# UBC-AWP/vision-sam3-yolo-lameless

Hardware: AMD Instinct MI355X
Metric: frames/sec (whole node) for YOLO+SAM3+DINOv3 feature extraction, 1080p clips (higher is better)
Workload: dtype f16; 1 GPU; BASELINE cfg#5, dense schedule: fused per-frame path on a synthetic 5 s @ 30 fps 1080p clip (150 unique BGR frames resident in HBM): YOLOv8-l detect (letterbox 384x640, NMS, scale_boxes; f16 plan) -> SAM (Hiera-B+ image encoder + FPN at 1024x1024, box-prompted mask decoder, 1080p mask + statistics + contour features) + DINOv3 ViT-L/16 embed (224x224) on EVERY frame; per-frame records packed, gathe; parallelism=one clip per GPU, 1 GPU(s), one gather per step, streams=7

## Files before the change

### vision-sam3-yolo-lameless_amd/csrc/attn.hip

```cpp
#include "common.h"
#include <type_traits>
#include <stdlib.h>

#ifdef LMX_DBG_TIMELINE
__device__ unsigned long long lmx_attn_tl[64 * 8 * 8];
extern "C" int lmx_dbg_get_attn_timeline(void* host, int64_t bytes) { return (int)hipMemcpyFromSymbol(host, HIP_SYMBOL(lmx_attn_tl), bytes); }
#define ATL(i) if (blockIdx.x == 0 && lane == 0 && tl_it < 64) lmx_attn_tl[(tl_it * 8 + wave) * 8 + (i)] = __builtin_readcyclecounter()
#else
#define ATL(i)
#endif
namespace {

struct Geo {
  int mode, Tq, Tk, Gh, Gw, ws, nWy, nWx, Gqh, Gqw, wsq;
};

__device__ __forceinline__ int64_t key_row(const Geo& g, int b, int t) {
  if (g.mode == 0) return (int64_t)b * g.Tk + t;
  const int nW = g.nWy * g.nWx;
  const int img = b / nW;
  const int w = b - img * nW;
  const int wy = w / g.nWx, wx = w - wy * g.nWx;
  const int ty = t / g.ws, tx = t - ty * g.ws;
  const int y = wy * g.ws + ty, x = wx * g.ws + tx;
// ... 691 lines not shown
  const int hd = p.hd;
  const half8_t zero8 = {0, 0, 0, 0, 0, 0, 0, 0};

  {
    const int r = lane >> 2, c0 = (lane & 3) * 2;
    const bool in = r < p.Tk;
    const int64_t row = key_row(geo, b, in ? r : 0);
    const bool pad = row < 0;
    half_t* dst = &Vs[wave][r * 64];
#pragma unroll
    for (int e = 0; e < 2; ++e) {
      const int c = c0 + e, d = c * 8;
      const bool ok = in && d < hd && (!pad || padv);
      const half_t* vp = (in && d < hd) ? (pad ? (padv ? padv + (int64_t)h * hd + d : V) : V + row * p.ldv + (int64_t)h * hd + d) : V;
      const half8_t vv = *reinterpret_cast<const half8_t*>(vp);
      *reinterpret_cast<half8_t*>(dst + ((c ^ (r & 7)) << 3)) = ok ? vv : zero8;
    }
  }
  const int64_t qrow = fr < p.Tq ? query_row(geo, b, fr) : -1;
  const bool kin = fr < p.Tk;
  const int64_t krow = key_row(geo, b, kin ? fr : 0);
  const bool kpad = krow < 0;
  half8_t qf[2], kf[2];
#pragma unroll
  for (int ks = 0; ks < 2; ++ks) {
    const int d = ks * 32 + fg * 8;
    const bool dq = qrow >= 0 && d < hd;
    const half8_t qv = *reinterpret_cast<const half8_t*>(Q + (dq ? qrow * p.ldq + (int64_t)h * hd + d : 0));
    qf[ks] = dq ? qv : zero8;
    const bool dk = kin && d < hd;
    const half_t* kp = dk ? (kpad ? (padk ? padk + (int64_t)h * hd + d : K) : K + krow * p.ldk + (int64_t)h * hd + d) : K;
    const half8_t kv = *reinterpret_cast<const half8_t*>(kp);
    kf[ks] = (dk && (!kpad || padk)) ? kv : zero8;
  }
  f32x4 sacc = {0.f, 0.f, 0.f, 0.f};
  sacc = __builtin_amdgcn_mfma_f32_16x16x32_f16(kf[0], qf[0], sacc, 0, 0, 0);
  sacc = __builtin_amdgcn_mfma_f32_16x16x32_f16(kf[1], qf[1], sacc, 0, 0, 0);
  const float sl2 = p.scale * 1.44269504088896340736f;
#pragma unroll
  for (int i = 0; i < 4; ++i)
    if (fg * 4 + i >= p.Tk) sacc[i] = -INFINITY;
  float mx = fmaxf(fmaxf(sacc[0], sacc[1]), fmaxf(sacc[2], sacc[3]));
  mx = fmaxf(mx, __shfl_xor(mx, 16, 64));
  mx = fmaxf(mx, __shfl_xor(mx, 32, 64));
  const float mb = mx * sl2;
  half8_t pf = zero8;
  float l = 0.f;
#pragma unroll
  for (int i = 0; i < 4; ++i) {
    const half_t e = (half_t)__builtin_amdgcn_exp2f(fmaf(sacc[i], sl2, -mb));
    pf[i] = e;
    l += (float)e;
  }
  l += __shfl_xor(l, 16, 64);
  l += __shfl_xor(l, 32, 64);
  const float inv = 1.0f / l;
  const int q4 = fr >> 2, p4 = fr & 3;
  const int r0 = fg * 4 + q4;
  half_t* O = reinterpret_cast<half_t*>(p.O);
#pragma unroll
  for (int db = 0; db < 4; ++db) {
    const int chunk = db * 2 + (p4 >> 1);
    const half4_t lo = lds_tr_read(&Vs[wave][r0 * 64 + ((chunk ^ (r0 & 7)) << 3) + (p4 & 1) * 4]);
    const half8_t vf = {lo[0], lo[1], lo[2], lo[3], 0, 0, 0, 0};
    f32x4 oacc = {0.f, 0.f, 0.f, 0.f};
    oacc = __builtin_amdgcn_mfma_f32_16x16x32_f16(vf, pf, oacc, 0, 0, 0);
    const int d = db * 16 + fg * 4;
    if (qrow >= 0 && d < hd) {
      const half4_t o = {(half_t)(oacc[0] * inv), (half_t)(oacc[1] * inv), (half_t)(oacc[2] * inv), (half_t)(oacc[3] * inv)};
      *reinterpret_cast<half4_t*>(O + qrow * p.ldo + (int64_t)h * hd + d) = o;
    }
  }
}

template <int KS>
__global__ __launch_bounds__(256) void relpos_tables_kernel(const lmx_attn_desc p, const Geo geo, const float* __restrict__ rh,
                                                            const float* __restrict__ rw, int S, half_t* __restrict__ out,
                                                            const int64_t items) {
  const int lane = threadIdx.x & 63, wave = threadIdx.x >> 6;
  const int fr = lane & 15, fg = lane >> 4;
  const int64_t item = (int64_t)blockIdx.x * 4 + wave;
  if (item >= items) return;
  const int line = (int)(item % S);
  const int axis = (int)((item / S) & 1);
  const int64_t bh = item / (2 * S);
  const int h = (int)(bh % p.H), b = (int)(bh / p.H);
  const int hd = p.hd;
  const float* R = axis ? rw : rh;
  const half_t* Q = reinterpret_cast<const half_t*>(p.Q);
  const half8_t zero8 = {0, 0, 0, 0, 0, 0, 0, 0};
  const int nblk = (S + 15) / 16;
  for (int mb = 0; mb < nblk; ++mb) {
    const int pos = mb * 16 + fr;
    const int t = axis ? pos * S + line : line * S + pos;
    const int64_t qrow = pos < S ? query_row(geo, b, t) : -1;
    half8_t qf[KS];
#pragma unroll
    for (int ks = 0; ks < KS; ++ks) {
      const int d = ks * 32 + fg * 8;
      const bool ok = qrow >= 0 && d < hd;
      const half8_t qv = *reinterpret_cast<const half8_t*>(Q + (ok ? qrow * p.ldq + (int64_t)h * hd + d : 0));
      qf[ks] = ok ? qv : zero8;
    }
    half_t* orow = out + ((bh * p.Tq) + (pos < S ? t : 0)) * (2 * S) + axis * S;
    for (int jb = 0; jb < nblk; ++jb) {
      const int j = jb * 16 + fr;
      f32x4 acc = {0.f, 0.f, 0.f, 0.f};
#pragma unroll
      for (int ks = 0; ks < KS; ++ks) {
        const int d = ks * 32 + fg * 8;
        const bool ok = j < S && d < hd;
        const float* rp = R + (ok ? (int64_t)(line - j + S - 1) * hd + d : 0);
        const f32x4 r0 = *reinterpret_cast<const f32x4*>(rp), r1 = *reinterpret_cast<const f32x4*>(rp + (ok ? 4 : 0));
        const half8_t rf = {(half_t)r0[0], (half_t)r0[1], (half_t)r0[2], (half_t)r0[3],
                            (half_t)r1[0], (half_t)r1[1], (half_t)r1[2], (half_t)r1[3]};
        acc = __builtin_amdgcn_mfma_f32_16x16x32_f16(ok ? rf : zero8, qf[ks], acc, 0, 0, 0);
      }
      const int j0 = jb * 16 + fg * 4;
      if (pos < S && j0 < S) {
        if (j0 + 3 < S && (S & 3) == 0) {
          const half4_t o = {(half_t)acc[0], (half_t)acc[1], (half_t)acc[2], (half_t)acc[3]};
          *reinterpret_cast<half4_t*>(orow + j0) = o;
        } else {
          for (int i = 0; i < 4 && j0 + i < S; ++i) orow[j0 + i] = (half_t)acc[i];
        }
      }
    }
  }
}


template <int QB, bool ONES>
__global__ __launch_bounds__(256, QB == 2 ? 2 : 3) void attn_sp_kernel(const lmx_attn_desc p, const Geo geo) {
  constexpr int RW = 64, CPR = 8, KB = 13, KROWS = KB * 16, VROWS = KROWS, NPASS = (KROWS + 31) / 32;
  __shared__ __attribute__((aligned(16))) half_t Ks[KROWS * RW];
  __shared__ __attribute__((aligned(16))) half_t Vs[VROWS * RW];
  const int tid = threadIdx.x, lane = tid & 63, wave = tid >> 6;
  const int fr = lane & 15, fg = lane >> 4;
  int bid;
  {
    const int n = gridDim.x, xcd = blockIdx.x & 7, idx = blockIdx.x >> 3, q = n >> 3, r = n & 7;
    bid = (xcd < r ? xcd * (q + 1) : r * (q + 1) + (xcd - r) * q) + idx;
  }
  const int h = bid % p.H, b = bid / p.H;
  const half_t* Q = reinterpret_cast<const half_t*>(p.Q);
  const half_t* K = reinterpret_cast<const half_t*>(p.K);
  const half_t* V = reinterpret_cast<const half_t*>(p.V);
  const half_t* padk = reinterpret_cast<const half_t*>(p.pad_k);
  const half_t* padv = reinterpret_cast<const half_t*>(p.pad_v);
  half_t* O = reinterpret_cast<half_t*>(p.O);
  const int hd = p.hd;
  const half8_t zero8 = {0, 0, 0, 0, 0, 0, 0, 0};

  {
    const int sc = tid & (CPR - 1), sk = tid / CPR;
    const int d = sc * 8;
    const int64_t hoff = (int64_t)h * hd + d;
#pragma unroll
    for (int half = 0; half < 2; ++half) {
      constexpr int H0 = 4;
      half8_t kst[H0], vst[H0];
#pragma unroll
      for (int j = 0; j < H0; ++j) {
        const int i = half * H0 + j;
        if (i >= NPASS) continue;
        const int t = sk + 32 * i;
        const bool in = (t < p.Tk) && (d < hd);
        const int64_t row = geo.mode == 0 ? (int64_t)b * p.Tk + (in ? t : 0) : key_row(geo, b, in ? t : 0);
        const bool pad = row < 0;
        const half_t* kp = pad ? (padk ? padk + hoff : K) : K + (in ? row * p.ldk + hoff : 0);
        const half_t* vp = pad ? (padv ? padv + hoff : V) : V + (in ? row * p.ldv + hoff : 0);
        const half8_t kv = *reinterpret_cast<const half8_t*>(kp);
        const half8_t vv = *reinterpret_cast<const half8_t*>(vp);
        kst[j] = (in && (!pad || padk)) ? kv : zero8;
        vst[j] = (in && (!pad || padv)) ? vv : zero8;
        if (ONES && sc == 7 && t < p.Tk) vst[j][7] = (half_t)1.0f;
      }
#pragma unroll
      for (int j = 0; j < H0; ++j) {
        const int i = half * H0 + j;
        if (i >= NPASS) continue;
        const int kk = sk + 32 * i;
        const int off = kk * RW + ((sc ^ (kk & (CPR - 1))) << 3);
        if (kk < KROWS) {
          *reinterpret_cast<half8_t*>(&Ks[off]) = kst[j];
          *reinterpret_cast<half8_t*>(&Vs[off]) = vst[j];
        }
      }
    }
  }
  __syncthreads();

  const float sl2 = p.scale * 1.44269504088896340736f;
  const int q4 = fr >> 2, p4 = fr & 3;
  const int nqb = (p.Tq + 15) / 16, npair = (nqb + QB - 1) / QB;
  for (int pr = wave; pr < npair; pr += 4) {
    half8_t qf[QB][2];
    int64_t qrow[QB];
#pragma unroll
    for (int qb = 0; qb < QB; ++qb) {
      const int tq = (pr * QB + qb) * 16 + fr;
      qrow[qb] = (tq < p.Tq) ? query_row(geo, b, tq) : -1;
#pragma unroll
      for (int ks = 0; ks < 2; ++ks) {
        const int d = ks * 32 + fg * 8;
        const bool ok = qrow[qb] >= 0 && d < hd;
        const half8_t qv = *reinterpret_cast<const half8_t*>(Q + (ok ? qrow[qb] * p.ldq + (int64_t)h * hd + d : 0));
        qf[qb][ks] = ok ? qv : zero8;
      }
    }
    f32x4 sacc[QB][KB];
#pragma unroll
    for (int qb = 0; qb < QB; ++qb)
#pragma unroll
      for (int kb = 0; kb < KB; ++kb) sacc[qb][kb] = f32x4{0.f, 0.f, 0.f, 0.f};
#pragma unroll
    for (int ks = 0; ks < 2; ++ks) {
      const int coff = (((ks << 2) + fg) ^ (fr & (CPR - 1))) << 3;
#pragma unroll
      for (int kb = 0; kb < KB; ++kb) {
        const half8_t kf = *reinterpret_cast<const half8_t*>(&Ks[(kb * 16 + fr) * RW + coff]);
#pragma unroll
        for (int qb = 0; qb < QB; ++qb) sacc[qb][kb] = __builtin_amdgcn_mfma_f32_16x16x32_f16(kf, qf[qb][ks], sacc[qb][kb], 0, 0, 0);
      }
    }
    half8_t pf[QB][7];
    float l_sum[QB];
#pragma unroll
    for (int qb = 0; qb < QB; ++qb) {
#pragma unroll
      for (int kb = 8; kb < KB; ++kb)
#pragma unroll
        for (int r = 0; r < 4; ++r)
          if (kb * 16 + fg * 4 + r >= p.Tk) sacc[qb][kb][r] = -INFINITY;
      float mx = fmaxf(fmaxf(sacc[qb][0][0], sacc[qb][0][1]), fmaxf(sacc[qb][0][2], sacc[qb][0][3]));
#pragma unroll
      for (int kb = 1; kb < KB; ++kb)
        mx = fmaxf(mx, fmaxf(fmaxf(sacc[qb][kb][0], sacc[qb][kb][1]), fmaxf(sacc[qb][kb][2], sacc[qb][kb][3])));
      mx = fmaxf(mx, __shfl_xor(mx, 16, 64));
      mx = fmaxf(mx, __shfl_xor(mx, 32, 64));
      const float mb = mx * sl2;
      float rs = 0.f;
      const half2_t ones2 = {(half_t)1.0f, (half_t)1.0f};
#pragma unroll
      for (int kb = 0; kb < KB + 1; ++kb)
#pragma unroll
        for (int r = 0; r < 4; r += 2) {
          half2_t e = {(half_t)0.0f, (half_t)0.0f};
          if (kb < KB) {
            const float e0 = __builtin_amdgcn_exp2f(fmaf(sacc[qb][kb][r], sl2, -mb));
            const float e1 = __builtin_amdgcn_exp2f(fmaf(sacc[qb][kb][r + 1], sl2, -mb));
            e = half2_t{(half_t)e0, (half_t)e1};
            if (!ONES) rs = __builtin_amdgcn_fdot2(e, ones2, rs, false);
          }
          pf[qb][kb >> 1][(kb & 1) * 4 + r] = e[0];
          pf[qb][kb >> 1][(kb & 1) * 4 + r + 1] = e[1];
        }
      l_sum[qb] = rs;
    }
    f32x4 oacc[QB][4];
#pragma unroll
    for (int qb = 0; qb < QB; ++qb)
#pragma unroll
      for (int db = 0; db < 4; ++db) oacc[qb][db] = f32x4{0.f, 0.f, 0.f, 0.f};
#pragma unroll
    for (int ks = 0; ks < 7; ++ks) {
#pragma unroll
      for (int db = 0; db < 4; ++db) {
        const int chunk = db * 2 + (p4 >> 1);
        const int r0 = ks * 32 + fg * 4 + q4, r1 = ks == 6 ? r0 : r0 + 16;
        const half4_t lo = lds_tr_read(&Vs[r0 * RW + ((chunk ^ (r0 & (CPR - 1))) << 3) + (p4 & 1) * 4]);
        const half4_t hi = lds_tr_read(&Vs[r1 * RW + ((chunk ^ (r1 & (CPR - 1))) << 3) + (p4 & 1) * 4]);
        const half8_t vf = {lo[0], lo[1], lo[2], lo[3], hi[0], hi[1], hi[2], hi[3]};
#pragma unroll
        for (int qb = 0; qb < QB; ++qb) oacc[qb][db] = __builtin_amdgcn_mfma_f32_16x16x32_f16(vf, pf[qb][ks], oacc[qb][db], 0, 0, 0);
      }
    }
#pragma unroll
    for (int qb = 0; qb < QB; ++qb) {
      float l;
      if (ONES) {
        l = __shfl(oacc[qb][3][3], 48 + fr, 64);
      } else {
        l = l_sum[qb];
        l += __shfl_xor(l, 16, 64);
        l += __shfl_xor(l, 32, 64);
      }
      const float inv = 1.0f / l;
      if (qrow[qb] < 0) continue;
#pragma unroll
      for (int db = 0; db < 4; ++db) {
        const int d = db * 16 + fg * 4;
        if (d >= hd) continue;
        half4_t o;
#pragma unroll
        for (int r = 0; r < 4; ++r) o[r] = (half_t)(oacc[qb][db][r] * inv);
        *reinterpret_cast<half4_t*>(O + qrow[qb] * p.ldo + (int64_t)h * hd + d) = o;
      }
    }
  }
}


template <bool ONES>
__global__ __launch_bounds__(512, 1) void attn_spp_kernel(const lmx_attn_desc p, const Geo geo, const int items) {
  constexpr int RW = 64, CPR = 8, KB = 13, ROWS = KB * 16, QB = 2, NWV = 8;
  constexpr int TEN = ROWS * RW * 2;
  constexpr int BUF = 3 * TEN;
  extern __shared__ __attribute__((aligned(16))) char smem[];
  const int tid = threadIdx.x, lane = tid & 63;
  const int wave = __builtin_amdgcn_readfirstlane(tid >> 6);
  const int fr = lane & 15, fg = lane >> 4;
  const int hd = p.hd, H_ = p.H, Tq_ = p.Tq, Tk_ = p.Tk, mode_ = geo.mode;
  const int64_t ldq_ = p.ldq, ldk_ = p.ldk, ldv_ = p.ldv;
  const int ws_ = geo.ws, wsq_ = geo.wsq, Gh_ = geo.Gh, Gw_ = geo.Gw, Gqh_ = geo.Gqh, Gqw_ = geo.Gqw, nWx_ = geo.nWx, nW_ = geo.nWy * geo.nWx;

  {
    const u32x4 z = {0u, 0u, 0u, 0u};
    for (int i = tid; i < 2 * BUF / 16; i += 512) *reinterpret_cast<u32x4*>(smem + i * 16) = z;
    __syncthreads();
    if (ONES)
      for (int i = tid; i < 2 * ROWS; i += 512) {
        const int bsel = i / ROWS, row = i - bsel * ROWS;
        half_t* v = reinterpret_cast<half_t*>(smem + bsel * BUF + 2 * TEN);
        v[row * RW + ((7 ^ (row & 7)) << 3) + 7] = (half_t)1.0f;
      }
  }

  const int xcd = blockIdx.x & 7, jx = blockIdx.x >> 3;
  const int nwg = ((int)gridDim.x + 7 - xcd) >> 3;
  const int iq = items >> 3, ir = items & 7;
  const int ibase = xcd < ir ? xcd * (iq + 1) : ir * (iq + 1) + (xcd - ir) * iq;
  const int icnt = iq + (xcd < ir ? 1 : 0);

  constexpr int NJ = 4;
  unsigned rel[3][NJ];
  int tyx[3][NJ];
#pragma unroll
  for (int ten = 0; ten < 3; ++ten)
#pragma unroll
    for (int m = 0; m < NJ; ++m) {
      const int j = wave + NWV * m;
      const int row = 8 * j + (lane >> 3);
      const int lc = (lane & 7) ^ (row & 7);
      const int d = lc * 8;
      const int T = ten == 0 ? Tq_ : Tk_;
      const int wsz = ten == 0 ? wsq_ : ws_;
      const int gw = ten == 0 ? Gqw_ : Gw_;
      const int64_t ld = ten == 0 ? ldq_ : (ten == 1 ? ldk_ : ldv_);
      const int ty = mode_ == 0 ? 0 : row / wsz, tx = mode_ == 0 ? row : row - ty * wsz;
      rel[ten][m] = (unsigned)((((int64_t)(mode_ == 0 ? row : ty * gw + tx)) * ld + d) * 2);
      tyx[ten][m] = ((j < 26 && row < T && d < hd) ? (1 << 30) : 0) | (d << 20) | (ty << 10) | tx;
    }
  const char* Qg = reinterpret_cast<const char*>(p.Q);
  const char* Kg = reinterpret_cast<const char*>(p.K);
  const char* Vg = reinterpret_cast<const char*>(p.V);
  const char* padk = reinterpret_cast<const char*>(p.pad_k);
  const char* padv = reinterpret_cast<const char*>(p.pad_v);
  int qty[QB], qtx[QB];
#pragma unroll
  for (int qb = 0; qb < QB; ++qb) {
    const int tq = (wave * QB + qb) * 16 + fr;
    qty[qb] = mode_ == 0 ? 0 : tq / wsq_;
    qtx[qb] = mode_ == 0 ? tq : tq - qty[qb] * wsq_;
  }

  auto issue = [&](int item, int bsel) {
    const int h = item % H_, b = item / H_;
    int img = b, wy = 0, wx = 0;
    if (mode_ != 0) {
      img = b / nW_;
      const int w = b - img * nW_;
      wy = w / nWx_;
      wx = w - wy * nWx_;
    }
    const int64_t hcol = (int64_t)h * hd * 2;
    const char *oq, *ok, *ov;
    int qy = 1 << 20, qx = 1 << 20, ky = 1 << 20, kx = 1 << 20;
    if (mode_ == 0) {
      oq = Qg + (int64_t)b * Tq_ * ldq_ * 2 + hcol;
      ok = Kg + (int64_t)b * Tk_ * ldk_ * 2 + hcol;
      ov = Vg + (int64_t)b * Tk_ * ldv_ * 2 + hcol;
    } else {
      const int64_t q0 = ((int64_t)img * Gqh_ + wy * wsq_) * Gqw_ + wx * wsq_;
      const int64_t k0 = ((int64_t)img * Gh_ + wy * ws_) * Gw_ + wx * ws_;
      oq = Qg + q0 * ldq_ * 2 + hcol;
      ok = Kg + k0 * ldk_ * 2 + hcol;
      ov = Vg + k0 * ldv_ * 2 + hcol;
      qy = Gqh_ - wy * wsq_, qx = Gqw_ - wx * wsq_, ky = Gh_ - wy * ws_, kx = Gw_ - wx * ws_;
    }
    const bool edge = qy < wsq_ || qx < wsq_ || ky < ws_ || kx < ws_;
    char* base = smem + bsel * BUF + wave * 1024;
#pragma unroll
    for (int ten = 0; ten < 3; ++ten) {
      const char* org = ten == 0 ? oq : (ten == 1 ? ok : ov);
      const char* pv = (ten == 1 ? padk : padv) + hcol;
#pragma unroll
      for (int m = 0; m < NJ; ++m) {
        if (wave + NWV * m >= 26) break;
        const int pl = tyx[ten][m];
        bool act = (pl >> 30) & 1;
        const char* src = org + rel[ten][m];
        if (edge) {
          const int ty = (pl >> 10) & 1023, tx = pl & 1023;
          if (ten == 0) {
            act = act && ty < qy && tx < qx;
          } else if (ty >= ky || tx >= kx) {
            src = pv + ((pl >> 20) & 1023) * 2;
          }
        }
        char* dst = base + ten * TEN + m * (NWV * 1024);
        if (act) __builtin_amdgcn_global_load_lds(reinterpret_cast<const void*>(src), (lds_ptr_t)dst, 16, 0, 0);
      }
    }
  };

  const float sl2 = p.scale * 1.44269504088896340736f;
  const int q4 = fr >> 2, p4 = fr & 3;
  const int nqb = (Tq_ + 15) / 16, npair = (nqb + QB - 1) / QB;
  __syncthreads();
  const bool early = wave < NWV / 2;
  if (jx < icnt) issue(ibase + jx, 0);
  asm volatile("s_waitcnt vmcnt(0)" ::: "memory");
  int bsel = 0;
#ifdef LMX_DBG_TIMELINE
  int tl_it = -1;
#endif
  for (int li = jx; li < icnt; li += nwg, bsel ^= 1) {
    const int item = ibase + li;
    const int h = item % p.H, b = item / p.H;
#ifdef LMX_DBG_TIMELINE
    ++tl_it;
#endif
    ATL(0);
    __syncthreads();
    ATL(1);
    const bool more = li + nwg < icnt;
    if (more && (early || wave >= npair)) issue(item + nwg, bsel ^ 1);
    ATL(2);
    const half_t* Qs = reinterpret_cast<const half_t*>(smem + bsel * BUF);
    const half_t* Ks = Qs + ROWS * RW;
    const half_t* Vs = Ks + ROWS * RW;
    const int pr = wave;
    if (pr < npair) {
      half8_t qf[QB][2];
      int64_t qrow[QB];
#pragma unroll
      for (int qb = 0; qb < QB; ++qb) {
        const int tq = (pr * QB + qb) * 16 + fr;
        if (mode_ == 0) {
          qrow[qb] = tq < Tq_ ? (int64_t)b * Tq_ + tq : -1;
        } else {
          const int img = b / nW_, w = b - img * nW_;
          const int wy = w / nWx_, wx = w - wy * nWx_;
          const int y = wy * wsq_ + qty[qb], x = wx * wsq_ + qtx[qb];
          qrow[qb] = (tq < Tq_ && y < Gqh_ && x < Gqw_) ? ((int64_t)img * Gqh_ + y) * Gqw_ + x : -1;
        }
        const int lr = tq < ROWS ? tq : ROWS - 1;
#pragma unroll
        for (int ks = 0; ks < 2; ++ks) qf[qb][ks] = *reinterpret_cast<const half8_t*>(&Qs[lr * RW + ((((ks << 2) + fg) ^ (lr & 7)) << 3)]);
      }
      f32x4 sacc[QB][KB];
#pragma unroll
      for (int qb = 0; qb < QB; ++qb)
#pragma unroll
        for (int kb = 0; kb < KB; ++kb) sacc[qb][kb] = f32x4{0.f, 0.f, 0.f, 0.f};
      {
        auto kread = [&](int i) {
          const int ks = i / KB, kb = i - ks * KB;
          return *reinterpret_cast<const half8_t*>(&Ks[(kb * 16 + fr) * RW + ((((ks << 2) + fg) ^ (fr & (CPR - 1))) << 3)]);
        };
        half8_t kring[3];
        kring[0] = kread(0);
        kring[1] = kread(1);
#pragma unroll
        for (int i = 0; i < 2 * KB; ++i) {
          if (i + 2 < 2 * KB) kring[(i + 2) % 3] = kread(i + 2);
          __builtin_amdgcn_sched_barrier(0);
          const int ks = i / KB, kb = i - ks * KB;
#pragma unroll
          for (int qb = 0; qb < QB; ++qb) sacc[qb][kb] = __builtin_amdgcn_mfma_f32_16x16x32_f16(kring[i % 3], qf[qb][ks], sacc[qb][kb], 0, 0, 0);
          __builtin_amdgcn_sched_barrier(0);
        }
      }
      if (more && !early) issue(item + nwg, bsel ^ 1);
      ATL(3);
      half8_t pf[QB][7];
      float l_sum[QB];
#pragma unroll
      for (int qb = 0; qb < QB; ++qb) {
#pragma unroll
        for (int kb = 8; kb < KB; ++kb)
          if (kb * 16 + 16 > Tk_) {
#pragma unroll
            for (int r = 0; r < 4; ++r)
              if (kb * 16 + fg * 4 + r >= Tk_) sacc[qb][kb][r] = -INFINITY;
          }
        float ma = vmax3(sacc[qb][0][0], sacc[qb][0][1], sacc[qb][0][2]);
        float mc = vmax3(sacc[qb][0][3], sacc[qb][1][0], sacc[qb][1][1]);
        ma = vmax3(ma, sacc[qb][1][2], sacc[qb][1][3]);
#pragma unroll
        for (int kb = 2; kb < KB; ++kb) {
          if (kb & 1)
            ma = vmax3(ma, sacc[qb][kb][0], sacc[qb][kb][1]), ma = vmax3(ma, sacc[qb][kb][2], sacc[qb][kb][3]);
          else
            mc = vmax3(mc, sacc[qb][kb][0], sacc[qb][kb][1]), mc = vmax3(mc, sacc[qb][kb][2], sacc[qb][kb][3]);
        }
        const float mx = row_max4(ma, mc);
        const float mb = mx * sl2;
        float rs = 0.f;
        const half2_t ones2 = {(half_t)1.0f, (half_t)1.0f};
#pragma unroll
        for (int kb = 0; kb < KB + 1; ++kb)
#pragma unroll
          for (int r = 0; r < 4; r += 2) {
            half2_t e = {(half_t)0.0f, (half_t)0.0f};
            if (kb < KB) {
              const float e0 = __builtin_amdgcn_exp2f(fmaf(sacc[qb][kb][r], sl2, -mb));
              const float e1 = __builtin_amdgcn_exp2f(fmaf(sacc[qb][kb][r + 1], sl2, -mb));
              e = half2_t{(half_t)e0, (half_t)e1};
              if (!ONES) rs = __builtin_amdgcn_fdot2(e, ones2, rs, false);
            }
            pf[qb][kb >> 1][(kb & 1) * 4 + r] = e[0];
            pf[qb][kb >> 1][(kb & 1) * 4 + r + 1] = e[1];
          }
        l_sum[qb] = rs;
      }
      ATL(4);
      f32x4 oacc[QB][4];
#pragma unroll
      for (int qb = 0; qb < QB; ++qb)
#pragma unroll
        for (int db = 0; db < 4; ++db) oacc[qb][db] = f32x4{0.f, 0.f, 0.f, 0.f};
      {
        u32x2_t vlo[3], vhi[3];
        auto vread = [&](int i, u32x2_t& lo, u32x2_t& hi) {
          const int ks = i >> 2, db = i & 3;
          const int chunk = db * 2 + (p4 >> 1);
          const int r0 = ks * 32 + fg * 4 + q4, r1 = ks == 6 ? r0 : r0 + 16;
          const unsigned a0 = (unsigned)(uintptr_t)(__attribute__((address_space(3))) const half_t*)&Vs[r0 * RW + ((chunk ^ (r0 & (CPR - 1))) << 3) + (p4 & 1) * 4];
          const unsigned a1 = (unsigned)(uintptr_t)(__attribute__((address_space(3))) const half_t*)&Vs[r1 * RW + ((chunk ^ (r1 & (CPR - 1))) << 3) + (p4 & 1) * 4];
          asm volatile("ds_read_b64_tr_b16 %0, %1" : "=v"(lo) : "v"(a0) : "memory");
          asm volatile("ds_read_b64_tr_b16 %0, %1" : "=v"(hi) : "v"(a1) : "memory");
        };
        vread(0, vlo[0], vhi[0]);
        vread(1, vlo[1], vhi[1]);
#pragma unroll
        for (int i = 0; i < 28; ++i) {
          if (i + 2 < 28) vread(i + 2, vlo[(i + 2) % 3], vhi[(i + 2) % 3]);
          if (i + 2 < 28)
            asm volatile("s_waitcnt lgkmcnt(4)" : "+v"(vlo[i % 3]), "+v"(vhi[i % 3])::"memory");
          else if (i + 1 < 28)
            asm volatile("s_waitcnt lgkmcnt(2)" : "+v"(vlo[i % 3]), "+v"(vhi[i % 3])::"memory");
          else
            asm volatile("s_waitcnt lgkmcnt(0)" : "+v"(vlo[i % 3]), "+v"(vhi[i % 3])::"memory");
          const u32x4_t w = {vlo[i % 3][0], vlo[i % 3][1], vhi[i % 3][0], vhi[i % 3][1]};
          const half8_t vf = __builtin_bit_cast(half8_t, w);
          const int ks = i >> 2, db = i & 3;
#pragma unroll
          for (int qb = 0; qb < QB; ++qb) oacc[qb][db] = __builtin_amdgcn_mfma_f32_16x16x32_f16(vf, pf[qb][ks], oacc[qb][db], 0, 0, 0);
          __builtin_amdgcn_sched_barrier(0);
        }
      }
      ATL(5);
      asm volatile("s_waitcnt vmcnt(0)" ::: "memory");
      ATL(6);
      half_t* O = reinterpret_cast<half_t*>(p.O);
#pragma unroll
      for (int qb = 0; qb < QB; ++qb) {
        float l;
        if (ONES) {
          l = __shfl(oacc[qb][3][3], 48 + fr, 64);
        } else {
          l = l_sum[qb];
          l += __shfl_xor(l, 16, 64);
          l += __shfl_xor(l, 32, 64);
        }
        const float inv = 1.0f / l;
        if (qrow[qb] < 0) continue;
#pragma unroll
        for (int db = 0; db < 4; ++db) {
          const int d = db * 16 + fg * 4;
          if (d >= hd) continue;
          half4_t o;
#pragma unroll
          for (int r = 0; r < 4; ++r) o[r] = (half_t)(oacc[qb][db][r] * inv);
          *reinterpret_cast<half4_t*>(O + qrow[qb] * p.ldo + (int64_t)h * hd + d) = o;
        }
      }
      ATL(7);
    } else {
      asm volatile("s_waitcnt vmcnt(0)" ::: "memory");
      ATL(7);
    }
  }
}

}

static int build_geo(const lmx_attn_desc& d, Geo& g);

extern "C" int lmx_k_relpos_tables(const lmx_attn_desc* dp, const float* rel_pos_h, const float* rel_pos_w, int S, void* out,
                                   lmx_stream_t stream) {
  LMX_REQUIRE(dp && rel_pos_h && rel_pos_w && out, "lmx_k_relpos_tables: null pointer");
  const lmx_attn_desc& d = *dp;
  LMX_REQUIRE(d.Q && d.B > 0 && d.H > 0 && d.Tq > 0 && d.hd % 8 == 0 && d.hd <= 96 && d.ldq % 8 == 0 && aligned16(d.Q),
              "lmx_k_relpos_tables: descriptor");
  LMX_REQUIRE(S > 0 && S * S == d.Tq, "lmx_k_relpos_tables: S=%d vs Tq=%d", S, d.Tq);
  Geo g{};
  const int rc = build_geo(d, g);
  if (rc) return rc;
  const int64_t items = (int64_t)d.B * d.H * 2 * S;
  const int64_t grid = (items + 3) / 4;
  LMX_REQUIRE(grid < (1ll << 31) && aligned16(rel_pos_h) && aligned16(rel_pos_w), "lmx_k_relpos_tables: size / alignment");
  hipStream_t st = reinterpret_cast<hipStream_t>(stream);
  if (d.hd <= 64)
    hipLaunchKernelGGL((relpos_tables_kernel<2>), dim3((unsigned)grid), dim3(256), 0, st, d, g, rel_pos_h, rel_pos_w, S,
                       reinterpret_cast<half_t*>(out), items);
  else
    hipLaunchKernelGGL((relpos_tables_kernel<3>), dim3((unsigned)grid), dim3(256), 0, st, d, g, rel_pos_h, rel_pos_w, S,
                       reinterpret_cast<half_t*>(out), items);
  return lmx_launch_check("relpos_tables_kernel");
}

enum AttnKernel { ATTN_SMALL, ATTN_SP, ATTN_SPP, ATTN_GP, ATTN_TILED };
struct AttnRoute {
  AttnKernel kernel;
  int QB = 1;
  bool ONES = false, REL = false, DMA = false;
  int HDW = 64, NWV = 4;
  unsigned grid = 0, block = 256;
  int lds = 0;
  int arg = 0;
};

static int attn_route(const lmx_attn_desc* dp, AttnRoute& r, Geo& g) {
  LMX_REQUIRE(dp != nullptr, "lmx_k_attention: null descriptor");
  const lmx_attn_desc& d = *dp;
  LMX_REQUIRE(d.Q && d.K && d.V && d.O, "lmx_k_attention: null Q/K/V/O");
  LMX_REQUIRE(d.B > 0 && d.H > 0 && d.Tq > 0 && d.Tk > 0, "lmx_k_attention: empty problem");
  LMX_REQUIRE(d.hd % 8 == 0 && d.hd > 0 && d.hd <= 96, "lmx_k_attention: head dim %d (need multiple of 8, <=96)", d.hd);
  LMX_REQUIRE(d.ldq % 8 == 0 && d.ldk % 8 == 0 && d.ldv % 8 == 0 && d.ldo % 4 == 0, "lmx_k_attention: strides");
  LMX_REQUIRE(aligned16(d.Q) && aligned16(d.K) && aligned16(d.V) && ((((uintptr_t)d.O) & 7) == 0),
              "lmx_k_attention: alignment");
  LMX_TRY(build_geo(d, g));
  static const int no_sp = lmx_env_set("LMX_ATTN_NO_SP"), sp_qb = lmx_env_int("LMX_ATTN_SP_QB", 2), no_spp = lmx_env_set("LMX_ATTN_NO_SPP");
  static const int no_dma = lmx_env_set("LMX_ATTN_NO_DMA"), no_lazy = lmx_env_set("LMX_ATTN_NO_LAZY");
  static const int no_gp = lmx_env_set("LMX_ATTN_NO_GP");
  static const int gp_waves = lmx_env_int("LMX_ATTN_GP_WAVES", 4);

  r = AttnRoute{};
  r.ONES = d.hd <= 56;
  const int64_t items = (int64_t)d.B * d.H;
  const bool narrow = !d.rel && d.hd <= 64;
  if (narrow && d.Tq <= 16 && d.Tk <= 16) {
    LMX_REQUIRE(items < (1ll << 31), "lmx_k_attention: grid too large");
    r.kernel = ATTN_SMALL;
    r.ONES = false;
    r.grid = (unsigned)((items + 3) / 4);
    r.arg = (int)items;
    return LMX_OK;
  }
  if (!no_sp && narrow && d.Tk > 128 && d.Tk <= 208 && d.Tq > 64 && d.Tq <= 208) {
    LMX_REQUIRE(items < (1ll << 31), "lmx_k_attention: grid too large");
    r.grid = (unsigned)items;
    if (!no_spp && items >= 64 && (d.mode == 0 || (d.pad_k && d.pad_v))) {
      r.kernel = ATTN_SPP;
      r.block = 512;
      r.lds = 2 * 3 * 208 * 64 * 2;
      r.arg = (int)items;
    } else {
      r.kernel = ATTN_SP;
      r.QB = sp_qb == 2 ? 2 : 1;
    }
    return LMX_OK;
  }
  const bool wide = d.hd > 64;
  const bool big = d.Tq > 64 && !wide;
  const int nQT = (d.Tq + (big ? 128 : 64) - 1) / (big ? 128 : 64);
  const int64_t nblk = items * nQT;
  LMX_REQUIRE(nblk < (1ll << 31), "lmx_k_attention: grid too large");
  if (d.rel)
    LMX_REQUIRE(d.rel_S > 0 && d.rel_S * d.rel_S == d.Tk && d.Tq == d.Tk, "lmx_k_attention: rel_S=%d does not match Tq=%d Tk=%d",
                d.rel_S, d.Tq, d.Tk);
  const bool dma = !no_dma && !wide && d.mode == 0 && !d.rel && big && d.Tk >= 256 && (int64_t)d.Tk * d.ldk * 2 < 0x7fff0000ll &&
                   (int64_t)d.Tk * d.ldv * 2 < 0x7fff0000ll;
  if (dma && !no_gp) {
    r.kernel = ATTN_GP;
    r.NWV = gp_waves == 8 ? 8 : 4;
    const int nQTw = (d.Tq + r.NWV * 32 - 1) / (r.NWV * 32);
    r.grid = (unsigned)(items * nQTw);
    r.block = r.NWV * 64;
    r.lds = 2 * 3 * 64 * 64 * 2;
    r.arg = no_lazy ? -nQTw : nQTw;
    return LMX_OK;
  }
  r.kernel = ATTN_TILED;
  r.QB = big ? 2 : 1;
  r.ONES = r.ONES && !d.rel;
  r.REL = d.rel != nullptr;
  r.DMA = dma;
  r.HDW = wide ? 96 : 64;
  r.grid = (unsigned)nblk;
  r.arg = no_lazy ? -nQT : nQT;
  return LMX_OK;
}

static constexpr int attn_key(int kernel, int QB, bool ONES, bool REL, bool DMA, int HDW, int NWV) {
  return (((((kernel * 4 + QB) * 2 + ONES) * 2 + REL) * 2 + DMA) * 128 + HDW) * 16 + NWV;
}

extern "C" int lmx_k_attention(const lmx_attn_desc* dp, lmx_stream_t stream) {
  AttnRoute r;
  Geo g{};
  LMX_TRY(attn_route(dp, r, g));
  const lmx_attn_desc& d = *dp;
  hipStream_t st = reinterpret_cast<hipStream_t>(stream);
  const dim3 block(r.block);
  dim3 grid(r.grid);
  if (r.kernel == ATTN_SPP) {
    int dev;
    LMX_TRY(lmx_stream_device(st, &dev));
    LMX_TRY(lmx_allow_lds(reinterpret_cast<const void*>(&attn_spp_kernel<true>), r.lds, dev));
    LMX_TRY(lmx_allow_lds(reinterpret_cast<const void*>(&attn_spp_kernel<false>), r.lds, dev));
    LMX_TRY(lmx_persistent_grid(r.grid, dev, &grid.x));
  }
#define LMX_SP(QB, ONES) \
  case attn_key(ATTN_SP, QB, ONES, false, false, 64, 4): hipLaunchKernelGGL((attn_sp_kernel<QB, ONES>), grid, block, 0, st, d, g); break
#define LMX_SPP(ONES) \
  case attn_key(ATTN_SPP, 1, ONES, false, false, 64, 4): hipLaunchKernelGGL((attn_spp_kernel<ONES>), grid, block, r.lds, st, d, g, r.arg); break
#define LMX_GP(ONES, NWV) \
  case attn_key(ATTN_GP, 1, ONES, false, false, 64, NWV): hipLaunchKernelGGL((attn_gp_kernel<ONES, NWV>), grid, block, r.lds, st, d, r.arg); break
#define LMX_TILED(QB, ONES, REL, DMA, HDW) \
  case attn_key(ATTN_TILED, QB, ONES, REL, DMA, HDW, 4): hipLaunchKernelGGL((attn_kernel<QB, ONES, REL, DMA, HDW>), grid, block, 0, st, d, g, r.arg); break
  switch (attn_key(r.kernel, r.QB, r.ONES, r.REL, r.DMA, r.HDW, r.NWV)) {
    case attn_key(ATTN_SMALL, 1, false, false, false, 64, 4): hipLaunchKernelGGL(attn_small_kernel, grid, block, 0, st, d, g, r.arg); break;
    LMX_SPP(true);
    LMX_SPP(false);
    LMX_SP(2, true);
    LMX_SP(1, true);
    LMX_SP(2, false);
    LMX_SP(1, false);
    LMX_TILED(1, false, true, false, 96);
    LMX_TILED(2, false, true, false, 64);
    LMX_TILED(1, false, true, false, 64);
    LMX_TILED(1, false, false, false, 96);
    LMX_GP(true, 8);
    LMX_GP(true, 4);
    LMX_GP(false, 8);
    LMX_GP(false, 4);
    LMX_TILED(2, true, false, true, 64);
    LMX_TILED(2, false, false, true, 64);
    LMX_TILED(2, true, false, false, 64);
    LMX_TILED(2, false, false, false, 64);
    LMX_TILED(1, true, false, false, 64);
    LMX_TILED(1, false, false, false, 64);
    default: LMX_REQUIRE(false, "lmx_k_attention: no kernel for route %d", (int)r.kernel);
  }
#undef LMX_SP
#undef LMX_SPP
#undef LMX_GP
#undef LMX_TILED
  static const char* const what[] = {"attn_small_kernel", "attn_sp_kernel", "attn_spp_kernel", "attn_gp_kernel", "attn_kernel"};
  return lmx_launch_check(what[r.kernel]);
}

extern "C" int lmx_h_attn_route(const lmx_attn_desc* dp, char* name, int cap) {
  AttnRoute r;
  Geo g{};
  LMX_TRY(attn_route(dp, r, g));
  const char* sums = r.ONES ? "ones" : "dot2";
  switch (r.kernel) {
    case ATTN_SMALL: LMX_ROUTE_NAME(name, cap, "small"); break;
    case ATTN_SP: LMX_ROUTE_NAME(name, cap, "sp_qb%d_%s", r.QB, sums); break;
    case ATTN_SPP: LMX_ROUTE_NAME(name, cap, "spp_%s", sums); break;
    case ATTN_GP: LMX_ROUTE_NAME(name, cap, "gp%d_%s", r.NWV, sums); break;
    case ATTN_TILED:
      LMX_ROUTE_NAME(name, cap, "tiled_q%d_%s%s%s_hd%d", r.QB, sums, r.REL ? "_rel" : "", r.DMA ? "_dma" : "", r.HDW);
      break;
  }
  return LMX_OK;
}

static int build_geo(const lmx_attn_desc& d, Geo& g) {
  g.mode = d.mode;
  g.Tq = d.Tq;
  g.Tk = d.Tk;
  if (d.mode == 1) {
    LMX_REQUIRE(d.ws > 0 && d.Gh > 0 && d.Gw > 0, "lmx_k_attention: window geometry");
    const int qs = d.q_stride > 0 ? d.q_stride : 1;
    LMX_REQUIRE(qs == 1 || qs == 2, "lmx_k_attention: q_stride %d", qs);
    LMX_REQUIRE(d.ws % qs == 0 && d.Gh % qs == 0 && d.Gw % qs == 0, "lmx_k_attention: q_stride must divide ws/Gh/Gw");
    g.Gh = d.Gh;
    g.Gw = d.Gw;
    g.ws = d.ws;
    g.nWy = (d.Gh + d.ws - 1) / d.ws;
    g.nWx = (d.Gw + d.ws - 1) / d.ws;
    g.Gqh = d.Gh / qs;
    g.Gqw = d.Gw / qs;
    g.wsq = d.ws / qs;
    LMX_REQUIRE(d.Tk == d.ws * d.ws && d.Tq == g.wsq * g.wsq, "lmx_k_attention: Tq/Tk do not match window size");
    LMX_REQUIRE(d.B % (g.nWy * g.nWx) == 0, "lmx_k_attention: B=%d not a multiple of windows per image %d", d.B,
                g.nWy * g.nWx);
    if (d.pad_k) LMX_REQUIRE(aligned16(d.pad_k), "lmx_k_attention: pad_k alignment");
    if (d.pad_v) LMX_REQUIRE(aligned16(d.pad_v), "lmx_k_attention: pad_v alignment");
  } else {
    LMX_REQUIRE(d.mode == 0, "lmx_k_attention: bad mode %d", d.mode);
  }
  return LMX_OK;
}
```

Baseline: 814.2 frames/s.

## Specialize SPP attention kernel on windowed mode and streamline item addressing

Adds a WIN template parameter to the persistent SPP attention kernel so non-windowed and windowed paths compile separately. Per-item division and modulo address decoding is replaced by incremental carry-based advancement of head, window and image indices. The async load issue is reworked so waves 0-3 load 16 rows each and wave 7 loops over the remaining 10 rows, with ballot masks replacing per-row validity bits. This reduces scalar and address arithmetic in the load issue and epilogue, at the cost of putting load issue on fewer waves and restricting SPP to cases where the query and key window geometry match.

```diff
diff --git a/vision-sam3-yolo-lameless_amd/csrc/attn.hip b/vision-sam3-yolo-lameless_amd/csrc/attn.hip
--- a/vision-sam3-yolo-lameless_amd/csrc/attn.hip
+++ b/vision-sam3-yolo-lameless_amd/csrc/attn.hip
@@ -1017,7 +1017,7 @@
 }
 
 
-template <bool ONES>
+template <bool ONES, bool WIN>
 __global__ __launch_bounds__(512, 1) void attn_spp_kernel(const lmx_attn_desc p, const Geo geo, const int items) {
   constexpr int RW = 64, CPR = 8, KB = 13, ROWS = KB * 16, QB = 2, NWV = 8;
   constexpr int TEN = ROWS * RW * 2;
@@ -1026,9 +1026,9 @@
   const int tid = threadIdx.x, lane = tid & 63;
   const int wave = __builtin_amdgcn_readfirstlane(tid >> 6);
   const int fr = lane & 15, fg = lane >> 4;
-  const int hd = p.hd, H_ = p.H, Tq_ = p.Tq, Tk_ = p.Tk, mode_ = geo.mode;
-  const int64_t ldq_ = p.ldq, ldk_ = p.ldk, ldv_ = p.ldv;
-  const int ws_ = geo.ws, wsq_ = geo.wsq, Gh_ = geo.Gh, Gw_ = geo.Gw, Gqh_ = geo.Gqh, Gqw_ = geo.Gqw, nWx_ = geo.nWx, nW_ = geo.nWy * geo.nWx;
+  const int hd = p.hd, H_ = p.H, Tq_ = p.Tq, Tk_ = p.Tk;
+  const int64_t ldq2 = p.ldq * 2, ldk2 = p.ldk * 2, ldv2 = p.ldv * 2, ldo2 = p.ldo * 2;
+  const int ws_ = WIN ? geo.ws : 1, Gh_ = WIN ? geo.Gh : 0, Gw_ = WIN ? geo.Gw : 0, nWx_ = WIN ? geo.nWx : 1, nWy_ = WIN ? geo.nWy : 1;
 
   {
     const u32x4 z = {0u, 0u, 0u, 0u};
@@ -1048,84 +1048,154 @@
   const int ibase = xcd < ir ? xcd * (iq + 1) : ir * (iq + 1) + (xcd - ir) * iq;
   const int icnt = iq + (xcd < ir ? 1 : 0);
 
-  constexpr int NJ = 4;
+  constexpr int NJ = 4, J7 = 16, N7 = 26 - J7;
   unsigned rel[3][NJ];
-  int tyx[3][NJ];
-#pragma unroll
-  for (int ten = 0; ten < 3; ++ten)
-#pragma unroll
-    for (int m = 0; m < NJ; ++m) {
-      const int j = wave + NWV * m;
-      const int row = 8 * j + (lane >> 3);
-      const int lc = (lane & 7) ^ (row & 7);
-      const int d = lc * 8;
-      const int T = ten == 0 ? Tq_ : Tk_;
-      const int wsz = ten == 0 ? wsq_ : ws_;
-      const int gw = ten == 0 ? Gqw_ : Gw_;
-      const int64_t ld = ten == 0 ? ldq_ : (ten == 1 ? ldk_ : ldv_);
-      const int ty = mode_ == 0 ? 0 : row / wsz, tx = mode_ == 0 ? row : row - ty * wsz;
-      rel[ten][m] = (unsigned)((((int64_t)(mode_ == 0 ? row : ty * gw + tx)) * ld + d) * 2);
-      tyx[ten][m] = ((j < 26 && row < T && d < hd) ? (1 << 30) : 0) | (d << 20) | (ty << 10) | tx;
-    }
+  int tyx[NJ];
+  const int dlane = ((lane & 7) ^ ((lane >> 3) & 7)) * 8;
+  const bool cin = ONES ? dlane < hd : true;
+  unsigned long long mq[NJ];
+#pragma unroll
+  for (int m = 0; m < NJ; ++m) {
+    const int j = NJ * (wave & 3) + m;
+    const int row = 8 * j + (lane >> 3);
+    const int ty = WIN ? row / ws_ : 0, tx = WIN ? row - ty * ws_ : row;
+    const int64_t tok = WIN ? ty * Gw_ + tx : row;
+    rel[0][m] = (unsigned)(tok * ldq2 + dlane * 2);
+    rel[1][m] = (unsigned)(tok * ldk2 + dlane * 2);
+    rel[2][m] = (unsigned)(tok * ldv2 + dlane * 2);
+    tyx[m] = (ty << 16) | tx;
+    mq[m] = __builtin_amdgcn_ballot_w64(row < Tq_ && cin);
+  }
+  const unsigned long long mfull = __builtin_amdgcn_ballot_w64(cin);
+  const int row7 = 8 * J7 + (lane >> 3);
+  const int ty7 = WIN ? row7 / ws_ : 0, tx7 = row7 - ty7 * ws_;
   const char* Qg = reinterpret_cast<const char*>(p.Q);
   const char* Kg = reinterpret_cast<const char*>(p.K);
   const char* Vg = reinterpret_cast<const char*>(p.V);
+  char* Og = reinterpret_cast<char*>(p.O);
   const char* padk = reinterpret_cast<const char*>(p.pad_k);
   const char* padv = reinterpret_cast<const char*>(p.pad_v);
   int qty[QB], qtx[QB];
 #pragma unroll
   for (int qb = 0; qb < QB; ++qb) {
     const int tq = (wave * QB + qb) * 16 + fr;
-    qty[qb] = mode_ == 0 ? 0 : tq / wsq_;
-    qtx[qb] = mode_ == 0 ? tq : tq - qty[qb] * wsq_;
-  }
-
-  auto issue = [&](int item, int bsel) {
-    const int h = item % H_, b = item / H_;
-    int img = b, wy = 0, wx = 0;
-    if (mode_ != 0) {
-      img = b / nW_;
-      const int w = b - img * nW_;
-      wy = w / nWx_;
-      wx = w - wy * nWx_;
-    }
-    const int64_t hcol = (int64_t)h * hd * 2;
+    const int ty = WIN ? tq / ws_ : 0;
+    qty[qb] = tq < Tq_ ? ty : 0x7fffffff;
+    qtx[qb] = tq - ty * ws_;
+  }
+
+  const int dh = nwg % H_, db = nwg / H_;
+  int dimg = db, dwy = 0, dwx = 0;
+  int nh, nimg, nwy = 0, nwx = 0;
+  {
+    const int it0 = ibase + jx;
+    nh = it0 % H_;
+    nimg = it0 / H_;
+    if (WIN) {
+      const int nW = nWy_ * nWx_;
+      dimg = db / nW;
+      const int r = db - dimg * nW;
+      dwy = r / nWx_;
+      dwx = r - dwy * nWx_;
+      const int b0 = nimg;
+      nimg = b0 / nW;
+      const int w = b0 - nimg * nW;
+      nwy = w / nWx_;
+      nwx = w - nwy * nWx_;
+    }
+  }
+  struct Item {
     const char *oq, *ok, *ov;
-    int qy = 1 << 20, qx = 1 << 20, ky = 1 << 20, kx = 1 << 20;
-    if (mode_ == 0) {
-      oq = Qg + (int64_t)b * Tq_ * ldq_ * 2 + hcol;
-      ok = Kg + (int64_t)b * Tk_ * ldk_ * 2 + hcol;
-      ov = Vg + (int64_t)b * Tk_ * ldv_ * 2 + hcol;
+    char* ob;
+    int hcol;
+    int ky, kx;
+    bool edge;
+  };
+  auto decode = [&]() {
+    Item it;
+    it.hcol = nh * hd * 2;
+    if (WIN) {
+      const int y0 = nwy * ws_, x0 = nwx * ws_;
+      const int64_t t0 = ((int64_t)nimg * Gh_ + y0) * Gw_ + x0;
+      it.oq = Qg + t0 * ldq2 + it.hcol;
+      it.ok = Kg + t0 * ldk2 + it.hcol;
+      it.ov = Vg + t0 * ldv2 + it.hcol;
+      it.ob = Og + t0 * ldo2 + it.hcol;
+      it.ky = Gh_ - y0;
+      it.kx = Gw_ - x0;
+      it.edge = it.ky < ws_ || it.kx < ws_;
     } else {
-      const int64_t q0 = ((int64_t)img * Gqh_ + wy * wsq_) * Gqw_ + wx * wsq_;
-      const int64_t k0 = ((int64_t)img * Gh_ + wy * ws_) * Gw_ + wx * ws_;
-      oq = Qg + q0 * ldq_ * 2 + hcol;
-      ok = Kg + k0 * ldk_ * 2 + hcol;
-      ov = Vg + k0 * ldv_ * 2 + hcol;
-      qy = Gqh_ - wy * wsq_, qx = Gqw_ - wx * wsq_, ky = Gh_ - wy * ws_, kx = Gw_ - wx * ws_;
-    }
-    const bool edge = qy < wsq_ || qx < wsq_ || ky < ws_ || kx < ws_;
-    char* base = smem + bsel * BUF + wave * 1024;
-#pragma unroll
-    for (int ten = 0; ten < 3; ++ten) {
-      const char* org = ten == 0 ? oq : (ten == 1 ? ok : ov);
-      const char* pv = (ten == 1 ? padk : padv) + hcol;
-#pragma unroll
-      for (int m = 0; m < NJ; ++m) {
-        if (wave + NWV * m >= 26) break;
-        const int pl = tyx[ten][m];
-        bool act = (pl >> 30) & 1;
-        const char* src = org + rel[ten][m];
-        if (edge) {
-          const int ty = (pl >> 10) & 1023, tx = pl & 1023;
-          if (ten == 0) {
-            act = act && ty < qy && tx < qx;
-          } else if (ty >= ky || tx >= kx) {
-            src = pv + ((pl >> 20) & 1023) * 2;
+      const int64_t q0 = (int64_t)nimg * Tq_, k0 = (int64_t)nimg * Tk_;
+      it.oq = Qg + q0 * ldq2 + it.hcol;
+      it.ok = Kg + k0 * ldk2 + it.hcol;
+      it.ov = Vg + k0 * ldv2 + it.hcol;
+      it.ob = Og + q0 * ldo2 + it.hcol;
+      it.ky = 1;
+      it.kx = 0x7fffffff;
+      it.edge = false;
+    }
+    return it;
+  };
+  auto advance = [&]() {
+    nh += dh;
+    int c = nh >= H_ ? 1 : 0;
+    nh -= c ? H_ : 0;
+    if (WIN) {
+      nwx += dwx + c;
+      c = nwx >= nWx_ ? 1 : 0;
+      nwx -= c ? nWx_ : 0;
+      nwy += dwy + c;
+      c = nwy >= nWy_ ? 1 : 0;
+      nwy -= c ? nWy_ : 0;
+    }
+    nimg += dimg + c;
+  };
+
+  auto issue = [&](const Item& it, int bsel) {
+    char* const img = smem + bsel * BUF;
+    auto dma = [&](const char* src, char* dst) {
+      __builtin_amdgcn_global_load_lds(reinterpret_cast<const void*>(src), (lds_ptr_t)dst, 16, 0, 0);
+    };
+    if (wave < 4) {
+      char* const base = img + wave * (NJ * 1024);
+      if (!WIN || !it.edge) {
+        if (__builtin_amdgcn_inverse_ballot_w64(mfull)) {
+#pragma unroll
+          for (int m = 0; m < NJ; ++m) dma(it.ok + rel[1][m], base + TEN + m * 1024);
+#pragma unroll
+          for (int m = 0; m < NJ; ++m) dma(it.ov + rel[2][m], base + 2 * TEN + m * 1024);
+        }
+#pragma unroll
+        for (int m = 0; m < NJ; ++m)
+          if (__builtin_amdgcn_inverse_ballot_w64(mq[m])) dma(it.oq + rel[0][m], base + m * 1024);
+      } else {
+#pragma unroll
+        for (int m = 0; m < NJ; ++m) {
+          const int ty = tyx[m] >> 16, tx = tyx[m] & 0xffff;
+          const bool in = ty < it.ky && tx < it.kx;
+          if (__builtin_amdgcn_inverse_ballot_w64(mq[m]) && in) dma(it.oq + rel[0][m], base + m * 1024);
+          if (__builtin_amdgcn_inverse_ballot_w64(mfull)) {
+            dma(in ? it.ok + rel[1][m] : padk + (it.hcol + dlane * 2), base + TEN + m * 1024);
+            dma(in ? it.ov + rel[2][m] : padv + (it.hcol + dlane * 2), base + 2 * TEN + m * 1024);
           }
         }
-        char* dst = base + ten * TEN + m * (NWV * 1024);
-        if (act) __builtin_amdgcn_global_load_lds(reinterpret_cast<const void*>(src), (lds_ptr_t)dst, 16, 0, 0);
+      }
+    } else if (wave == NWV - 1) {
+      int row = row7, ty = ty7, tx = tx7;
+      char* dst = img + J7 * 1024;
+#pragma unroll 1
+      for (int m = 0; m < N7; ++m, row += 8, dst += 1024) {
+        const int64_t tok = WIN ? ty * Gw_ + tx : row;
+        const bool in = WIN ? ty < it.ky && tx < it.kx : true;
+        if (row < Tq_ && cin && in) dma(it.oq + (tok * ldq2 + dlane * 2), dst);
+        if (row < Tk_ && cin) {
+          dma(in ? it.ok + (tok * ldk2 + dlane * 2) : padk + (it.hcol + dlane * 2), dst + TEN);
+          dma(in ? it.ov + (tok * ldv2 + dlane * 2) : padv + (it.hcol + dlane * 2), dst + 2 * TEN);
+        }
+        if (WIN) {
+          tx += 8;
+          if (tx >= ws_) tx -= ws_, ++ty;
+        }
       }
     }
   };
@@ -1134,16 +1204,16 @@
   const int q4 = fr >> 2, p4 = fr & 3;
   const int nqb = (Tq_ + 15) / 16, npair = (nqb + QB - 1) / QB;
   __syncthreads();
-  const bool early = wave < NWV / 2;
-  if (jx < icnt) issue(ibase + jx, 0);
+  Item nx = decode();
+  if (jx < icnt) issue(nx, 0);
   asm volatile("s_waitcnt vmcnt(0)" ::: "memory");
   int bsel = 0;
 #ifdef LMX_DBG_TIMELINE
   int tl_it = -1;
 #endif
   for (int li = jx; li < icnt; li += nwg, bsel ^= 1) {
-    const int item = ibase + li;
-    const int h = item % p.H, b = item / p.H;
+    char* const cob = nx.ob;
+    const int cky = nx.ky, ckx = nx.kx;
 #ifdef LMX_DBG_TIMELINE
     ++tl_it;
 #endif
@@ -1151,7 +1221,9 @@
     __syncthreads();
     ATL(1);
     const bool more = li + nwg < icnt;
-    if (more && (early || wave >= npair)) issue(item + nwg, bsel ^ 1);
+    advance();
+    nx = decode();
+    if (more) issue(nx, bsel ^ 1);
     ATL(2);
     const half_t* Qs = reinterpret_cast<const half_t*>(smem + bsel * BUF);
     const half_t* Ks = Qs + ROWS * RW;
@@ -1159,18 +1231,9 @@
     const int pr = wave;
     if (pr < npair) {
       half8_t qf[QB][2];
-      int64_t qrow[QB];
 #pragma unroll
       for (int qb = 0; qb < QB; ++qb) {
         const int tq = (pr * QB + qb) * 16 + fr;
-        if (mode_ == 0) {
-          qrow[qb] = tq < Tq_ ? (int64_t)b * Tq_ + tq : -1;
-        } else {
-          const int img = b / nW_, w = b - img * nW_;
-          const int wy = w / nWx_, wx = w - wy * nWx_;
-          const int y = wy * wsq_ + qty[qb], x = wx * wsq_ + qtx[qb];
-          qrow[qb] = (tq < Tq_ && y < Gqh_ && x < Gqw_) ? ((int64_t)img * Gqh_ + y) * Gqw_ + x : -1;
-        }
         const int lr = tq < ROWS ? tq : ROWS - 1;
 #pragma unroll
         for (int ks = 0; ks < 2; ++ks) qf[qb][ks] = *reinterpret_cast<const half8_t*>(&Qs[lr * RW + ((((ks << 2) + fg) ^ (lr & 7)) << 3)]);
@@ -1198,7 +1261,6 @@
           __builtin_amdgcn_sched_barrier(0);
         }
       }
-      if (more && !early) issue(item + nwg, bsel ^ 1);
       ATL(3);
       half8_t pf[QB][7];
       float l_sum[QB];
@@ -1280,7 +1342,6 @@
       ATL(5);
       asm volatile("s_waitcnt vmcnt(0)" ::: "memory");
       ATL(6);
-      half_t* O = reinterpret_cast<half_t*>(p.O);
 #pragma unroll
       for (int qb = 0; qb < QB; ++qb) {
         float l;
@@ -1292,7 +1353,8 @@
           l += __shfl_xor(l, 32, 64);
         }
         const float inv = 1.0f / l;
-        if (qrow[qb] < 0) continue;
+        if (!(qty[qb] < cky && qtx[qb] < ckx)) continue;
+        char* const orow = cob + (int64_t)(qty[qb] * Gw_ + qtx[qb]) * ldo2;
 #pragma unroll
         for (int db = 0; db < 4; ++db) {
           const int d = db * 16 + fg * 4;
@@ -1300,7 +1362,7 @@
           half4_t o;
 #pragma unroll
           for (int r = 0; r < 4; ++r) o[r] = (half_t)(oacc[qb][db][r] * inv);
-          *reinterpret_cast<half4_t*>(O + qrow[qb] * p.ldo + (int64_t)h * hd + d) = o;
+          *reinterpret_cast<half4_t*>(orow + d * 2) = o;
         }
       }
       ATL(7);
@@ -1343,6 +1405,7 @@
   AttnKernel kernel;
   int QB = 1;
   bool ONES = false, REL = false, DMA = false;
+  bool WIN = false;
   int HDW = 64, NWV = 4;
   unsigned grid = 0, block = 256;
   int lds = 0;
@@ -1379,8 +1442,9 @@
   if (!no_sp && narrow && d.Tk > 128 && d.Tk <= 208 && d.Tq > 64 && d.Tq <= 208) {
     LMX_REQUIRE(items < (1ll << 31), "lmx_k_attention: grid too large");
     r.grid = (unsigned)items;
-    if (!no_spp && items >= 64 && (d.mode == 0 || (d.pad_k && d.pad_v))) {
+    if (!no_spp && items >= 64 && (d.mode == 0 || (d.pad_k && d.pad_v && g.wsq == g.ws && g.Gqh == g.Gh && g.Gqw == g.Gw))) {
       r.kernel = ATTN_SPP;
+      r.WIN = d.mode != 0;
       r.block = 512;
       r.lds = 2 * 3 * 208 * 64 * 2;
       r.arg = (int)items;
@@ -1436,14 +1500,19 @@
   if (r.kernel == ATTN_SPP) {
     int dev;
     LMX_TRY(lmx_stream_device(st, &dev));
-    LMX_TRY(lmx_allow_lds(reinterpret_cast<const void*>(&attn_spp_kernel<true>), r.lds, dev));
-    LMX_TRY(lmx_allow_lds(reinterpret_cast<const void*>(&attn_spp_kernel<false>), r.lds, dev));
+    LMX_TRY(lmx_allow_lds(reinterpret_cast<const void*>(&attn_spp_kernel<true, true>), r.lds, dev));
+    LMX_TRY(lmx_allow_lds(reinterpret_cast<const void*>(&attn_spp_kernel<true, false>), r.lds, dev));
+    LMX_TRY(lmx_allow_lds(reinterpret_cast<const void*>(&attn_spp_kernel<false, true>), r.lds, dev));
+    LMX_TRY(lmx_allow_lds(reinterpret_cast<const void*>(&attn_spp_kernel<false, false>), r.lds, dev));
     LMX_TRY(lmx_persistent_grid(r.grid, dev, &grid.x));
   }
 #define LMX_SP(QB, ONES) \
   case attn_key(ATTN_SP, QB, ONES, false, false, 64, 4): hipLaunchKernelGGL((attn_sp_kernel<QB, ONES>), grid, block, 0, st, d, g); break
-#define LMX_SPP(ONES) \
-  case attn_key(ATTN_SPP, 1, ONES, false, false, 64, 4): hipLaunchKernelGGL((attn_spp_kernel<ONES>), grid, block, r.lds, st, d, g, r.arg); break
+#define LMX_SPP(ONES)                                                                                                 \
+  case attn_key(ATTN_SPP, 1, ONES, false, false, 64, 4):                                                              \
+    if (r.WIN) hipLaunchKernelGGL((attn_spp_kernel<ONES, true>), grid, block, r.lds, st, d, g, r.arg);                \
+    else hipLaunchKernelGGL((attn_spp_kernel<ONES, false>), grid, block, r.lds, st, d, g, r.arg);                     \
+    break
 #define LMX_GP(ONES, NWV) \
   case attn_key(ATTN_GP, 1, ONES, false, false, 64, NWV): hipLaunchKernelGGL((attn_gp_kernel<ONES, NWV>), grid, block, r.lds, st, d, r.arg); break
 #define LMX_TILED(QB, ONES, REL, DMA, HDW) \
```

After: 819.2 frames/s (median of 6 runs). Within noise of the previous version (+0.6%).
